# scwolof/gp_grief

Measured on AMD Instinct MI355X. Metric: CG iters/sec + Kron-matvec achieved HBM GB/s, 4D RBF grid 200^4, higher is better.
Workload: dtype f64

## Files before the change

### gp_grief_amd/csrc/gg_internal.h

```cpp
#pragma once

#include <hip/hip_runtime.h>

#include <algorithm>
#include <cstdint>
#include <cstdio>
#include <stdexcept>
#include <string>
#include <vector>

#include "../../include/gp_grief_amd.h"

namespace gg {

struct Error : std::runtime_error {
  int code;
  Error(int c, const std::string& m) : std::runtime_error(m), code(c) {}
};

void set_last_error(const std::string& msg);

#define GG_HIP(expr)                                                              \
  do {                                                                            \
    hipError_t e_ = (expr);                                                       \
    if (e_ != hipSuccess)                                                         \
      throw ::gg::Error(GG_ERR_RUNTIME, std::string("HIP error '") +              \
                                           hipGetErrorString(e_) + "' at " +     \
                                           __FILE__ + ":" + std::to_string(__LINE__) + \
                                           " in " #expr);                         \
  } while (0)

#define GG_REQUIRE(cond, code, msg)                 \
  do {                                              \
    if (!(cond)) throw ::gg::Error((code), (msg));  \
  } while (0)

template <class F>
int guard(F&& body) {
  try {
    body();
    return GG_OK;
  } catch (const Error& e) {
    set_last_error(e.what());
    return e.code;
  } catch (const std::bad_alloc&) {
    set_last_error("host allocation failed");
    return GG_ERR_RUNTIME;
  } catch (const std::exception& e) {
    set_last_error(e.what());
    return GG_ERR_RUNTIME;
  }
}

inline hipStream_t as_stream(gg_stream s) { return reinterpret_cast<hipStream_t>(s); }

#define GG_LAUNCH_CHECK() GG_HIP(hipGetLastError())

constexpr int kWave = 64;

inline int64_t ceil_div(int64_t a, int64_t b) { return (a + b - 1) / b; }

inline bool aligned16(const void* p) { return (reinterpret_cast<uintptr_t>(p) & 15) == 0; }

inline void check_status(int st) {
  if (st == GG_OK) return;
  char buf[512];
  gg_last_error(buf, sizeof buf);
  throw Error(st, buf);
}

constexpr int kXWinMax = 8;
constexpr int kXWinDefault = 8;
struct CgScalars {
  double rho;
  double rho_prev;
  double pq;
  double alpha;
  double beta;
  double tol;
  double bnorm;
  int iters;
  int done;
  int first;
  int pending;
  double rq, qq;
  int repair;
  int xpend;
  double xc[2];
  const double* xp[2];
  int xh;
  int xs;
  double xsc;
  const double* xsp;
  int cancels;
  double cancel_tol;
  int wk;
  int wn;
  int wnext;
  int warm;
  int wa[kXWinMax];
  double wc[kXWinMax + 1];
  const double* wp[kXWinMax + 1];
  int sreg, scnt;
  double scoef[kXWinMax];
  const double* sdir[kXWinMax];
  double beta_p;
  int rstored;
  const double* rp_cur;
  const double* rp_prev;
};

struct MpFuse {
  double* r = nullptr;
  const double* q_old = nullptr;
  double qshift = 0.0;
  double* p_out = nullptr;
  const CgScalars* sc = nullptr;
  double* rr_part = nullptr;
  int64_t rr_cap = 0;
  int64_t* pro_blocks = nullptr;
  int64_t pqo_stride = 0;
  double* sx = nullptr;
  const double* sp = nullptr;
  int64_t sn = 0, schunk = 0;
  int xdefer = 0;
  int xwin = 0;
  int64_t soff = 0;
  int64_t soff_h1 = 0, sn_h1 = 0;
  double* first_dst = nullptr;
  const double* er = nullptr;
  int64_t pstride = 0;
  double* ep_out = nullptr;
  double* ex = nullptr;
  const double* coef = nullptr;
  double* blk_q_out = nullptr;
  bool rderive = false;
  const double* pprev = nullptr;
};

struct OutMap {
  int identity;
  int64_t cg, gs, mi, cr, hs, as;
  int push = 0;
  int64_t self_off = 0;
  double* const* peers = nullptr;
  static OutMap ident() { return OutMap{1, 1, 0, 1, 1, 0, 0}; }
};

constexpr int kVecBlocks = 2048;
constexpr int kVecThreads = 256;

inline int vec_blocks(int64_t n) {
  const int64_t want = ceil_div(std::max<int64_t>(n / 2, 1), kVecThreads);
  return (int)std::min<int64_t>(kVecBlocks, std::max<int64_t>(want, 1));
}

struct KronDiag {
  int d;
  int64_t m[16];
  int64_t off[16];
};

inline KronDiag make_diag(int d, const int64_t* m, int64_t* n_out) {
  GG_REQUIRE(d >= 1 && d <= 16, GG_ERR_VALUE, "1 <= d <= 16 factors supported");
  GG_REQUIRE(m != nullptr, GG_ERR_VALUE, "NULL argument");
  KronDiag kd{};
  kd.d = d;
  int64_t n = 1, off = 0;
  for (int k = 0; k < d; ++k) {
    GG_REQUIRE(m[k] >= 1, GG_ERR_VALUE, "empty factor");
    kd.m[k] = m[k];
    kd.off[k] = off;
    off += m[k];
    n *= m[k];
  }
  *n_out = n;
  return kd;
}

// ... 125 lines not shown
```

### gp_grief_amd/csrc/gg_kronb.hip

```cpp
#include <algorithm>
#include <cmath>
#include <cstdlib>
#include <vector>

#include "gg_internal.h"

namespace gg {

typedef double bd4 __attribute__((ext_vector_type(4)));

constexpr int kBlkMaxD = 6;
constexpr int kBlkModeWaves = 12;
constexpr int kBlkPairWaves = 4;

struct BlockOp {
  int d = 0;
  int64_t m[kBlkMaxD] = {}, h[kBlkMaxD] = {};
  int64_t e[kBlkMaxD] = {};
  int64_t nb = 0, n = 0;
  double* frag[kBlkMaxD][2] = {};
  int KS[kBlkMaxD] = {}, JT[kBlkMaxD] = {};
  bool T4[kBlkMaxD] = {};
  int pTF = 0;
  int cus = 256;
// ... 682 lines not shown
#pragma unroll
        for (int r = 0; r < 4; ++r)
          stq(cvalid, a.Y, (cbase + (int64_t)(16 * t + 4 * r) * a.inner) * 8, o_e, acc[t][r]);
      stq(cvalid, a.Y, (cbase + (int64_t)16 * TF * a.inner) * 8, o_e, acc4);
      cur_next(cc);
    }
    sg0 = sg1;
  }
  if (KIND == 1 || KIND == 4) {
    __shared__ double red[2 * W];
#pragma unroll
    for (int off = 32; off > 0; off >>= 1) {
      rr_acc += __shfl_xor(rr_acc, off, 64);
      pqo_acc += __shfl_xor(pqo_acc, off, 64);
    }
    if (lane == 0) {
      red[wave] = rr_acc;
      red[W + wave] = pqo_acc;
    }
    __syncthreads();
    if (threadIdx.x == 0) {
      double s0 = 0.0, s1 = 0.0;
      for (int w = 0; w < W; ++w) {
        s0 += red[w];
        s1 += red[W + w];
      }
      if (a.rr_part != nullptr) {
        a.rr_part[blockIdx.x] = s0;
        if (a.pqo_stride > 0) a.rr_part[a.pqo_stride + blockIdx.x] = s1;
      }
    }
  }
}

struct PairArgs {
  const double* X;
  double* Y;
  const double* f3S;
  const double* f3T;
  const double* f2S;
  const double* f2T;
  int64_t nslab;
  int64_t spb;
  int64_t blk0;
  const double* P;
  double shift;
  double* partials;
  int64_t pstride;
  const int* skip;
  const CgScalars* sc;
  double* sx;
  int64_t soff, sn, soff_h1, sn_h1, sstep;
  int64_t sreg_len;
};

template <int R>
__device__ __forceinline__ double bcast_group(double v) {
  constexpr int pat = (R << 7) | 0x13;
  const int lo = __builtin_amdgcn_ds_swizzle(__double2loint(v), pat);
  const int hi = __builtin_amdgcn_ds_swizzle(__double2hiint(v), pat);
  return __hiloint2double(hi, lo);
}

template <int TF, int J0, int NJ, bool TJ, int EPI = -1, int PF = 4, bool NT = false>
__device__ __forceinline__ void pair_gemm2(const PairArgs& A, int64_t sbyte, const double* f2,
                                           const bd4 (&W)[TF][NJ > 0 ? NJ : 1],
                                           const double (&Wta)[NJ > 0 ? NJ : 1],
                                           const double (&Wj)[TF], const double Wc, double& pq,
                                           double& qq) {
  constexpr int H = 16 * TF + 4;
  constexpr int KS = 4 * TF + 1;
  constexpr int64_t FS = (int64_t)(TF + 1) * 64 * 8;
  const int lane = threadIdx.x & 63;
  const int n16 = lane & 15, kq = lane >> 4, l3 = lane & 3, b4 = (lane >> 2) & 3;
  uint32_t o_f = (uint32_t)(lane * 8);
  uint32_t o_z = (uint32_t)(((n16 >> 2) * 4 * H + 4 * kq + (n16 & 3)) * 8);
  uint32_t o_zt = (uint32_t)((16 * b4 + 4 * kq + l3) * 8);
  asm volatile("" : "+v"(o_f), "+v"(o_z), "+v"(o_zt));
  auto zb = [&](int i0, int a0) -> int64_t { return sbyte + ((int64_t)a0 * H + 4 * i0) * 8; };
  const bool epi = EPI < 0 ? A.P != nullptr : EPI != 0;
  const double sh = A.shift;
  auto bfull = [&](int s, int u) -> double {
    return s < 4 * TF ? W[s >> 2][u][s & 3] : Wta[u];
  };
  auto btail = [&](int s) -> double {
    if (s >= 4 * TF) return Wc;
    switch (s & 3) {
      case 0: return bcast_group<0>(Wj[s >> 2]);
      case 1: return bcast_group<1>(Wj[s >> 2]);
      case 2: return bcast_group<2>(Wj[s >> 2]);
      default: return bcast_group<3>(Wj[s >> 2]);
    }
  };
  auto put = [&](int64_t ub, uint32_t vo, double z, double p) {
    double q = z;
    if (epi) {
      q = fma(sh, p, q);
      pq = fma(p, q, pq);
      qq = fma(q, q, qq);
    }
    stuq<NT>(A.Y, ub, vo, q);
  };
#pragma unroll 1
  for (int ti = 0; ti < TF; ++ti) {
    bd4 Z[NJ > 0 ? NJ : 1];
    double Zt = 0.0;
#pragma unroll
// ... 319 lines not shown
  __shared__ __attribute__((aligned(16))) double ring[NS * R::STAGE];
  if (A.skip != nullptr && *A.skip) return;
  const int lane = threadIdx.x & 63;
  const int wave = __builtin_amdgcn_readfirstlane(threadIdx.x >> 6);
  const int sl = wave >> 1;
  const int64_t G = gridDim.x;
  const int64_t nunit = A.nslab / SPW;
  const int nmine = __builtin_amdgcn_readfirstlane(
      (int)((nunit - (int64_t)blockIdx.x + G - 1) / G));
  uint32_t dlane[R::DPW];
  uint32_t dlds[R::DPW];
#pragma unroll
  for (int j = 0; j < R::DPW; ++j) {
    const int i = wave * R::DPW + j;
    if (i < SPW * R::XI) {
      const int xs = i / R::XI, xi = i % R::XI;
      const int t = 2 * xi + (lane >> 5);
      const int row = min(16 * t + (lane & 15), H - 1);
      dlane[j] = (uint32_t)(xs * SB + (row * 4 + 2 * ((lane >> 4) & 1)) * 8);
      dlds[j] = (uint32_t)(xs * R::XD + xi * 128);
    } else {
      const int f = min(i - SPW * R::XI, R::FI - 1);
      dlane[j] = (uint32_t)((2 * f * 64 + 2 * lane) * 8);
      dlds[j] = (uint32_t)(R::FD + f * 128);
    }
  }
  auto src_at = [&](int it) {
    const int64_t slab = ((int64_t)blockIdx.x + (int64_t)it * G) * SPW;
    PairSlabSrc p;
    p.xoff = uni64(slab * SB);
    const int par = __builtin_amdgcn_readfirstlane((int)((slab / A.spb + A.blk0) & 1));
    p.f3 = par ? A.f3T : A.f3S;
    return p;
  };
  auto issue = [&](const PairSlabSrc& p, int st, int slot) {
    const char* xb = ubase(A.X, p.xoff + (int64_t)st * H * 32);
    const char* fbs = ubase(p.f3, (int64_t)st * FSK);
    double* dst = ring + slot * R::STAGE;
#pragma unroll
    for (int j = 0; j < R::DPW; ++j) {
      const int i = wave * R::DPW + j;
      const char* src = i < SPW * R::XI ? xb : fbs;
      __builtin_amdgcn_global_load_lds(
          reinterpret_cast<const __attribute__((address_space(1))) void*>(
              reinterpret_cast<uintptr_t>(src + dlane[j])),
          (__attribute__((address_space(3))) void*)(dst + dlds[j]), 16, 0, 0);
    }
  };
  double sc0 = 0.0, sc1 = 0.0;
  const double* sp0 = nullptr;
  const double* sp1 = nullptr;
  double* sxo = nullptr;
  int64_t slen = 0;
  double wcf[kXWinMax];
  const double* wdir[kXWinMax];
  int wcnt = 0;
  if (SIDE & 4) {
    if (A.sc->warm && !A.sc->done) {
      const int64_t off = (int64_t)A.sc->sreg * A.sreg_len;
      slen = max((int64_t)0, min(A.sn - off, A.sreg_len));
      wcnt = A.sc->scnt;
#pragma unroll
      for (int t = 0; t < kXWinMax; ++t) {
        wcf[t] = A.sc->scoef[t];
        wdir[t] = A.sc->sdir[t] + off;
      }
      sxo = A.sx + off;
    }
  } else if (SIDE & 1) {
    const int xh = A.sc->xh;
    if (xh < 2 && !A.sc->done) {
      const int64_t off = xh ? A.soff_h1 : A.soff;
      slen = xh ? A.sn_h1 : A.sn;
      sc0 = A.sc->xc[0];
      sc1 = A.sc->xc[1];
      sp0 = A.sc->xp[0] + off;
      sp1 = A.sc->xp[1] + off;
      sxo = A.sx + off;
    }
  }
  auto side_chunk = [&](int64_t slot) {
    const int64_t q0 = slot * A.sstep;
    const int64_t q1 = min(slen, q0 + A.sstep);
    constexpr int kSB = 16;
    for (int64_t e0 = q0 + 2 * lane; e0 < q1; e0 += kSB * 128) {
      double2 xv[kSB], a[kSB], b[kSB];
#pragma unroll
      for (int u = 0; u < kSB; ++u) {
        const int64_t e = e0 + (int64_t)u * 128;
        if (e + 1 < q1) {
          xv[u] = ld2g(sxo + e);
          a[u] = ld2g(sp0 + e);
          b[u] = ld2g(sp1 + e);
        }
      }
#pragma unroll
      for (int u = 0; u < kSB; ++u) {
        const int64_t e = e0 + (int64_t)u * 128;
        if (e + 1 < q1) {
          double2 o;
          o.x = xv[u].x + (sc0 * a[u].x + sc1 * b[u].x);
          o.y = xv[u].y + (sc0 * a[u].y + sc1 * b[u].y);
          st2g(sxo + e, o);
        }
      }
    }
  };
  auto side_chunk_win = [&](int64_t slot) {
    const int64_t q0 = slot * A.sstep;
    const int64_t q1 = min(slen, q0 + A.sstep);
    constexpr int kWB = 4;
    for (int64_t e0 = q0 + 2 * lane; e0 < q1; e0 += kWB * 128) {
      double2 xv[kWB], a[kXWinMax][kWB];
#pragma unroll
      for (int u = 0; u < kWB; ++u) {
        const int64_t e = e0 + (int64_t)u * 128;
        if (e + 1 < q1) xv[u] = ld2g(sxo + e);
      }
#pragma unroll
      for (int t = 0; t < kXWinMax; ++t)
        if (t < wcnt)
#pragma unroll
          for (int u = 0; u < kWB; ++u) {
            const int64_t e = e0 + (int64_t)u * 128;
            if (e + 1 < q1) a[t][u] = ld2g(wdir[t] + e);
          }
#pragma unroll
      for (int u = 0; u < kWB; ++u) {
        const int64_t e = e0 + (int64_t)u * 128;
        if (e + 1 < q1) {
          double2 s = {0.0, 0.0};
#pragma unroll
          for (int t = 0; t < kXWinMax; ++t)
            if (t < wcnt) {
              s.x += wcf[t] * a[t][u].x;
              s.y += wcf[t] * a[t][u].y;
            }
          double2 o;
          o.x = xv[u].x + s.x;
          o.y = xv[u].y + s.y;
          st2g(sxo + e, o);
        }
      }
    }
  };
  PairSlabSrc cur = src_at(0);
#pragma unroll
  for (int j = 0; j + 1 < NS; ++j) issue(cur, min(j, R::KS - 1), j);
  double pq = 0.0, qq = 0.0;
  int cslot = 0;
  for (int it = 0; it < nmine; ++it) {
    const int64_t slab = ((int64_t)blockIdx.x + (int64_t)it * G) * SPW + sl;
    const bool nv = it + 1 < nmine;
    const PairSlabSrc nxt = nv ? src_at(it + 1) : cur;
    const int role = (wave + it) & 1;
    if (role == 0)
      pair_slab_lds<TF, SPW, EPI, 0, JA, true, (SIDE & 2) != 0>(A, slab, sl, cslot, it == 0, cur, nxt, nv, ring,
                                               issue, pq, qq);
    else
      pair_slab_lds<TF, SPW, EPI, JA, TF - JA, false, (SIDE & 2) != 0>(A, slab, sl, cslot, it == 0, cur, nxt, nv,
                                                      ring, issue, pq, qq);
    if ((SIDE & 4) && slen > 0)
      side_chunk_win(((int64_t)blockIdx.x + (int64_t)it * G) * R::NW + wave);
    else if ((SIDE & 1) && slen > 0)
      side_chunk(((int64_t)blockIdx.x + (int64_t)it * G) * R::NW + wave);
    cslot = (cslot + R::KS) % NS;
    cur = nxt;
  }
  blk_wait_vm<0>();
  if (A.partials != nullptr) {
    __syncthreads();
    double* red = ring;
#pragma unroll
    for (int off = 32; off > 0; off >>= 1) {
      pq += __shfl_xor(pq, off, 64);
      qq += __shfl_xor(qq, off, 64);
    }
    if (lane == 0) {
      red[wave] = pq;
      red[R::NW + wave] = qq;
    }
    __syncthreads();
    if (threadIdx.x == 0) {
      double s0 = 0.0, s1 = 0.0;
      for (int w = 0; w < R::NW; ++w) {
        s0 += red[w];
        s1 += red[R::NW + w];
      }
      A.partials[blockIdx.x] = s0;
      A.partials[A.pstride + blockIdx.x] = 0.0;
      A.partials[2 * A.pstride + blockIdx.x] = s1;
    }
  }
}

typedef void (*blk_mode_fn)(ModeArgs);
typedef void (*blk_pair_fn)(PairArgs);



template <int KIND>
static blk_mode_fn mode_fn(int JT, bool T4) {
#define GG_BLK_MODE(jt)                                                    \
  case jt:                                                                 \
    return T4 ? blk_mode_kernel<jt, true, KIND> : blk_mode_kernel<jt, false, KIND>;
  switch (JT) {
    GG_BLK_MODE(1)
    GG_BLK_MODE(2)
    GG_BLK_MODE(3)
    GG_BLK_MODE(4)
    GG_BLK_MODE(5)
    GG_BLK_MODE(6)
    GG_BLK_MODE(7)
    default: return nullptr;
  }
#undef GG_BLK_MODE
}
// ... 378 lines not shown
      a.rr_part = cg->rr_part;
      GG_REQUIRE(grid <= cg->rr_cap, GG_ERR_VALUE, "prologue partial array too short");
      if (cg->pro_blocks != nullptr) *cg->pro_blocks = grid;
    } else if (kind == 2) {
      a.sc = cg->sc;
      a.sx = cg->sx;
      const int64_t sn = cg->sn;
      const int64_t H = block_side_half(sn);
      a.soff = 0;
      a.sn = std::min(H, sn);
      a.soff_h1 = a.sn;
      a.sn_h1 = sn - a.sn;
      const int64_t slots = a.ngroups * W;
      a.sstep = 2 * ceil_div(std::max<int64_t>(std::max(a.sn, a.sn_h1), 1), 2 * slots);
      GG_REQUIRE(a.sstep <= 128 * (int64_t)a.KS, GG_ERR_VALUE,
                 "block CG: x side job larger than its k-steps");
    }
    const blk_mode_fn fn = select_mode(kind, B->JT[k], B->T4[k], (int)B->h[k], B->fast);
    const size_t lds = (size_t)B->KS[k] * B->JT[k] * 64 * sizeof(double);
    hipLaunchKernelGGL(fn, dim3(grid), dim3(64 * W), lds, stream, a);
    GG_LAUNCH_CHECK();
    if (k == 0 && d == 3 && side && !pair_side)
      launch_x_half(cg->sx, cg->sn, block_side_half(cg->sn), cg->sc, stream);
    if (ev) GG_HIP(hipEventRecord(ev[++pos], stream));
    src = chain;
  }
  PairArgs p{};
  p.X = src;
  p.Y = cgp >= 2 ? cg->blk_q_out : y;
  const int k3 = d - 1, k2 = d - 2;
  p.f3S = B->frag[k3][0];
  p.f3T = B->frag[k3][1];
  p.f2S = B->frag[k2][0];
  p.f2T = B->frag[k2][1];
  p.spb = B->nb / (B->e[k3] * B->e[k2]);
  p.nslab = p.spb * nblk;
  p.blk0 = blk0;
  p.skip = skip;
  const int grid = pair_grid(B, nblk);
  if (cgp >= 2) {
    p.P = cg->p_out;
    p.shift = shift;
    p.partials = dot_partials;
    p.pstride = cg->pstride;
  } else if (shift != 0.0) {
    p.P = x;
    p.shift = shift;
  }
  if (pair_side && win) {
    p.sc = cg->sc;
    p.sx = cg->sx;
    p.sn = cg->sn;
    p.sreg_len = xwin_region(cg->sn, cg->xwin);
    const int64_t slots = p.nslab / B->pair_spw * 2 * B->pair_spw;
    p.sstep = 2 * ceil_div(std::max<int64_t>(p.sreg_len, 1), 2 * slots);
  } else if (pair_side) {
    p.sc = cg->sc;
    p.sx = cg->sx;
    const int64_t sn = cg->sn;
    const int64_t H = block_side_half(sn);
    p.soff = 0;
    p.sn = std::min(H, sn);
    p.soff_h1 = p.sn;
    p.sn_h1 = sn - p.sn;
    const int64_t slots = p.nslab / B->pair_spw * 2 * B->pair_spw;
    p.sstep = 2 * ceil_div(std::max<int64_t>(std::max(p.sn, p.sn_h1), 1), 2 * slots);
  }
  hipLaunchKernelGGL(select_pair(B->pTF, B->pair_lds, B->pair_spw, p.P != nullptr, pair_side,
                                 B->epi_nt && (pair_side || cgp == 3), win),
                     dim3(grid), dim3(B->pair_lds ? 128 * B->pair_spw : 64 * kBlkPairWaves), 0,
                     stream, p);
  GG_LAUNCH_CHECK();
  if (ev) GG_HIP(hipEventRecord(ev[++pos], stream));
  if (n_partials) *n_partials = (cgp >= 2) ? grid : 0;
}

int64_t block_side_half(int64_t n) { return 2 * ceil_div(n, (int64_t)4); }

bool block_pair_side(const BlockOp* B) { return B != nullptr && B->pair_lds; }

bool block_rderive_ok(const BlockOp* B) {
  if (B == nullptr || B->d < 3 || !B->pro_nt) return false;
  const int JT = B->JT[0];
  return B->T4[0] && B->h[0] == 16 * (JT - 1) + 4 && B->fast && mode_fast_fn<5>(JT) != nullptr;
}

bool block_efficient(const BlockOp* B) {
  if (B == nullptr) return false;
  const int d = B->d;
  return B->e[d - 1] == B->h[d - 1] && B->e[d - 2] == B->h[d - 2];
}

}
```

### gp_grief_amd/csrc/gg_vec.hip

```cpp
#include <cmath>
#include <map>
#include <vector>

#include "gg_internal.h"

namespace gg {

__global__ __launch_bounds__(kVecThreads) void dot_partials_kernel(const double* __restrict__ x,
                                                                   const double* __restrict__ y,
                                                                   int64_t n,
                                                                   double* __restrict__ partials) {
  double acc = 0.0;
  const int64_t stride = (int64_t)gridDim.x * blockDim.x;
  const int64_t n2 = n / 2;
  const double2* x2 = reinterpret_cast<const double2*>(x);
  const double2* y2 = reinterpret_cast<const double2*>(y);
  for (int64_t i = (int64_t)blockIdx.x * blockDim.x + threadIdx.x; i < n2; i += stride) {
    const double2 a = x2[i], b = y2[i];
    acc = fma(a.x, b.x, acc);
    acc = fma(a.y, b.y, acc);
  }
  if (blockIdx.x == 0 && threadIdx.x == 0 && (n & 1)) acc = fma(x[n - 1], y[n - 1], acc);
  const double s = block_sum(acc);
  if (threadIdx.x == 0) partials[blockIdx.x] = s;
// ... 454 lines not shown
    sc->wnext = 0;
    sc->warm = 0;
    for (int r = 0; r < kXWinMax; ++r) sc->wa[r] = 0;
    sc->beta_p = 0.0;
    sc->rstored = 1;
    sc->rp_cur = sc->rp_prev = nullptr;
    sc->done = (s == 0.0 || !(sqrt(s) >= sc->tol)) ? 1 : 0;
  }
}

void scalars_clear(CgScalars* sc) {
  GG_HIP(hipMemset(sc, 0, sizeof(CgScalars)));
  const char* e = knob("GG_CG_CANCEL_TOL");
  if (e) {
    const double t = atof(e);
    GG_HIP(hipMemcpy(&sc->cancel_tol, &t, sizeof(double), hipMemcpyHostToDevice));
  }
}
}

struct gg_cg {
  const gg_kron* K = nullptr;
  double shift = 0.0;
  int64_t n = 0;
  double *r = nullptr, *p = nullptr, *q = nullptr, *mv_work = nullptr;
  double* p2 = nullptr;
  double* p3 = nullptr;
  double* p4 = nullptr;
  double* first_dst = nullptr;
  bool fused = true;
  int fusion = 0;
  int xdefer = 2;
  double* partials = nullptr;
  double* rr_part = nullptr;
  int64_t rr_count = 0;
  int rq = 1;
  gg::CgScalars* sc = nullptr;
  gg::CgScalars* sc_host = nullptr;
  const double* b = nullptr;
  double* x = nullptr;
  int64_t mv_partials = 0;
  bool await_finish = false;
  bool profiling = false;
  std::vector<hipEvent_t> events;
  size_t events_used = 0;
  const gg::BlockOp* blk = nullptr;
  int basis = 1;
  bool block = false;
  double* xb = nullptr;
  double* q2 = nullptr;
  int64_t rblk0 = 0, rnblk = -1;
  bool restart = false;
  int xwin = 0;
  int xmode = 0;
  double* ring[gg::kXWinMax + 1] = {};
  int pcur = 0;
  double *q_c = nullptr, *q2_c = nullptr;
  bool rder_ok = true;
  bool rder = false;
  double* pprev_buf() const {
    const int ns = nring();
    return ring[(pcur + ns - 1) % ns];
  }
  int launches() const { return block ? gg::block_launches(blk) : gg::kron_d(K); }
  int nring() const { return xmode == 3 ? xwin + 1 : 4; }
  int64_t nvec() const { return (block && rnblk < 0) ? gg::block_n(blk) : n; }
  void reset_buffers() {
    p = ring[0];
    p2 = ring[1];
    p3 = ring[2];
    p4 = ring[3];
    q = q_c;
    q2 = q2_c;
    pcur = 0;
  }
  void rotate_dirs() {
    if (xmode == 3) {
      const int ns = nring();
      pcur = (pcur + 1) % ns;
      p = ring[pcur];
      p2 = ring[(pcur + 1) % ns];
    } else if (xmode == 2) {
      double* cur = p;
      double* o2 = p3;
      p = p2;
      p2 = p4;
      p3 = cur;
      p4 = o2;
    } else if (xmode == 1) {
      double* old_ = p3;
      p3 = p;
      p = p2;
      p2 = old_;
    } else {
      std::swap(p, p2);
    }
  }
};

namespace gg {
static int cg_xwin_knob() {
  const char* e = knob("GG_CG_XWIN");
  const int k = e ? atoi(e) : kXWinDefault;
  return k < 2 ? 0 : std::min(k, kXWinMax);
}
static int64_t cg_extra_dirs(int K) { return K >= 2 ? std::max(0, K + 1 - 4) : 0; }
int64_t xwin_region(int64_t n, int K) { return 2 * ceil_div(n, 2 * (int64_t)K); }
}

extern "C" {

int gg_dot(const double* x_dev, const double* y_dev, int64_t n, double* out_host,
           gg_stream stream) {
  return gg::guard([&] {
    GG_REQUIRE(x_dev && y_dev && out_host && n >= 0, GG_ERR_VALUE, "bad argument");
    hipStream_t s = gg::as_stream(stream);
    double* buf = nullptr;
    GG_HIP(hipMallocAsync(&buf, (gg::kVecBlocks + 1) * sizeof(double), s));
    const int nb = gg::vec_blocks(n);
    if (gg::aligned16(x_dev) && gg::aligned16(y_dev)) {
      gg::launch_dot_partials(x_dev, y_dev, n, buf, nb, s);
    } else {
      hipLaunchKernelGGL(gg::dot_partials_unaligned_kernel, dim3(nb), dim3(gg::kVecThreads), 0,
                         s, x_dev, y_dev, n, buf);
      GG_LAUNCH_CHECK();
    }
    gg::launch_reduce_to(buf, nb, buf + gg::kVecBlocks, s);
    GG_HIP(hipMemcpyAsync(out_host, buf + gg::kVecBlocks, sizeof(double),
                          hipMemcpyDeviceToHost, s));
    GG_HIP(hipFreeAsync(buf, s));
    GG_HIP(hipStreamSynchronize(s));
  });
}

int gg_axpby(double a, const double* x_dev, double b, double* y_dev, int64_t n,
             gg_stream stream) {
  return gg::guard([&] {
    GG_REQUIRE(x_dev && y_dev && n >= 0, GG_ERR_VALUE, "bad argument");
    if (n == 0) return;
    hipLaunchKernelGGL(gg::axpby_kernel, dim3(gg::vec_blocks(2 * n)), dim3(gg::kVecThreads),
                       0, gg::as_stream(stream), a, x_dev, b, y_dev, n);
    GG_LAUNCH_CHECK();
  });
}

static int64_t cg_vec_pad() {
  const char* e = gg::knob("GG_CG_VEC_PAD");
  const int64_t v = e ? atoll(e) : 0;
  return v > 0 ? 2 * (v / 2) : 0;
}
static int64_t cg_vec_stride(int64_t n) { return (n + 31) / 32 * 32 + cg_vec_pad(); }
constexpr int64_t kCgAlignSlack = 32;

static int64_t cg_layout_elems(const gg_kron* K, int64_t n, int64_t* extra_off = nullptr,
                               int* xwin = nullptr, int64_t* vstride = nullptr) {
  const gg::BlockOp* B = gg::kron_block(K);
  const int64_t vs = cg_vec_stride(B ? std::max(n, gg::block_n(B)) : n);
// ... 9 lines not shown
static thread_local std::map<const gg_kron*, int64_t> t_cg_sized;

int gg_cg_work_elems(const gg_kron* K, int64_t* elems) {
  return gg::guard([&] {
    GG_REQUIRE(K && elems, GG_ERR_VALUE, "NULL argument");
    gg::knobs_reload();
    const int64_t n = gg::kron_n(K);
    *elems = cg_layout_elems(K, n);
    t_cg_sized[K] = *elems;
  });
}

int gg_cg_work_elems_blocks(const gg_kron* K, int64_t nblk, int64_t* elems) {
  return gg::guard([&] {
    GG_REQUIRE(K && elems, GG_ERR_VALUE, "NULL argument");
    const gg::BlockOp* B = gg::kron_block(K);
    GG_REQUIRE(B != nullptr, GG_ERR_VALUE, "the operator has no parity-block basis");
    GG_REQUIRE(nblk >= 1 && nblk <= ((int64_t)1 << gg::block_d(B)), GG_ERR_VALUE,
               "block count outside 1..2^d");
    gg::knobs_reload();
    const int w = gg::block_pair_side(B) ? gg::cg_xwin_knob() : 0;
    *elems = kCgAlignSlack + (7 + gg::cg_extra_dirs(w)) * cg_vec_stride(nblk * gg::block_nb(B));
  });
}

int gg_cg_create_blocks(const gg_kron* K, int64_t blk0, int64_t nblk, double shift,
                        double* work_dev, gg_cg** out) {
  return gg::guard([&] {
    GG_REQUIRE(K && work_dev && out, GG_ERR_VALUE, "NULL argument");
    const gg::BlockOp* B = gg::kron_block(K);
    GG_REQUIRE(B != nullptr, GG_ERR_VALUE, "the operator has no parity-block basis");
    GG_REQUIRE(gg::block_d(B) >= 3, GG_ERR_VALUE, "the block-sharded CG needs d >= 3");
    GG_REQUIRE(blk0 >= 0 && nblk >= 1 && blk0 + nblk <= ((int64_t)1 << gg::block_d(B)),
               GG_ERR_VALUE, "block range outside the 2^d blocks");
    GG_REQUIRE((reinterpret_cast<uintptr_t>(work_dev) & 15) == 0, GG_ERR_VALUE,
               "the CG workspace must be 16-byte aligned");
    const int64_t n = nblk * gg::block_nb(B);
    gg_cg* cg = new gg_cg();
    try {
      cg->K = K;
      cg->shift = shift;
      cg->n = n;
      const int64_t vs = cg_vec_stride(n);
      work_dev = reinterpret_cast<double*>((reinterpret_cast<uintptr_t>(work_dev) + 255) &
                                           ~static_cast<uintptr_t>(255));
      cg->r = work_dev;
      cg->p = work_dev + vs;
      cg->q = work_dev + 2 * vs;
      cg->p2 = work_dev + 3 * vs;
      cg->p3 = work_dev + 4 * vs;
      cg->p4 = work_dev + 5 * vs;
      cg->q2 = work_dev + 6 * vs;
      cg->xwin = gg::block_pair_side(B) ? gg::cg_xwin_knob() : 0;
      cg->ring[0] = cg->p;
      cg->ring[1] = cg->p2;
      cg->ring[2] = cg->p3;
      cg->ring[3] = cg->p4;
      for (int i = 0; i < gg::cg_extra_dirs(cg->xwin); ++i) cg->ring[4 + i] = work_dev + (7 + i) * vs;
      cg->q_c = cg->q;
      cg->q2_c = cg->q2;
      cg->blk = B;
      cg->basis = 1;
      cg->rblk0 = blk0;
      cg->rnblk = nblk;
      cg->fused = true;
      const char* rde = gg::knob("GG_CG_RDERIVE");
      cg->rder_ok = !(rde && atoi(rde) == 0);
      cg->mv_partials = gg::block_partials_needed(B);
      GG_HIP(hipMalloc(&cg->partials,
                       std::max<int64_t>(gg::kVecBlocks, 3 * cg->mv_partials) * sizeof(double)));
      cg->rr_count = gg::block_prologue_blocks(B);
      GG_HIP(hipMalloc(&cg->rr_part, 2 * cg->rr_count * sizeof(double)));
      GG_HIP(hipMemset(cg->rr_part, 0, 2 * cg->rr_count * sizeof(double)));
      GG_HIP(hipMalloc(&cg->sc, sizeof(gg::CgScalars)));
      GG_HIP(hipHostMalloc(&cg->sc_host, sizeof(gg::CgScalars), hipHostMallocDefault));
      gg::scalars_clear(cg->sc);
    } catch (...) {
      gg_cg_destroy(cg);
      throw;
    }
    *out = cg;
  });
}

int gg_cg_create(const gg_kron* K, double shift, double* work_dev, gg_cg** out) {
  return gg::guard([&] {
    GG_REQUIRE(K && work_dev && out, GG_ERR_VALUE, "NULL argument");
    int64_t nr = 0, nc = 0, we = 0;
    gg_kron_shape(K, 0, &nr, &nc, &we);
    GG_REQUIRE(nr == nc, GG_ERR_VALUE, "CG needs a square operator");
    gg_cg* cg = new gg_cg();
    try {
      cg->K = K;
      cg->shift = shift;
      cg->n = nr;
      int64_t vs = 0;
      const int64_t need = cg_layout_elems(K, nr, nullptr, nullptr, &vs);
      const auto sized = t_cg_sized.find(K);
      GG_REQUIRE(sized == t_cg_sized.end() || need <= sized->second, GG_ERR_VALUE,
                 "the CG workspace was sized (gg_cg_work_elems) under another GG_* snapshot: "
                 "call gg_cg_work_elems again before gg_cg_create");
      if (sized != t_cg_sized.end()) t_cg_sized.erase(sized);
      GG_REQUIRE((reinterpret_cast<uintptr_t>(work_dev) & 7) == 0, GG_ERR_VALUE,
                 "the CG workspace must hold doubles (8-byte aligned)");
      const bool base16 = (reinterpret_cast<uintptr_t>(work_dev) & 15) == 0;
      work_dev = reinterpret_cast<double*>((reinterpret_cast<uintptr_t>(work_dev) + 255) &
                                           ~static_cast<uintptr_t>(255));
      cg->r = work_dev;
      cg->p = work_dev + vs;
      cg->q = work_dev + 2 * vs;
      cg->p2 = work_dev + 3 * vs;
      cg->p3 = work_dev + 4 * vs;
      cg->p4 = work_dev + 5 * vs;
      cg->mv_work = work_dev + 6 * vs;
      if (gg::kron_d(K) % 2 == 1) cg->first_dst = cg->mv_work + gg::kron_work_elems(K, false);
      cg->blk = gg::kron_block(K);
      int64_t extra_off = 0;
      int xwin = 0;
      cg_layout_elems(K, nr, &extra_off, &xwin);
      cg->ring[0] = cg->p;
      cg->ring[1] = cg->p2;
      cg->ring[2] = cg->p3;
      cg->ring[3] = cg->p4;
      cg->q_c = cg->q;
      if (cg->blk != nullptr) {
        cg->xb = work_dev + 6 * vs;
        cg->q2 = work_dev + 7 * vs;
        cg->q2_c = cg->q2;
        const char* be = gg::knob("GG_CG_BASIS");
        cg->basis = be ? (atoi(be) != 0 ? 1 : 0) : (gg::block_efficient(cg->blk) ? 1 : 0);
        cg->xwin = gg::block_pair_side(cg->blk) ? xwin : 0;
        for (int i = 0; i < gg::cg_extra_dirs(xwin); ++i)
          cg->ring[4 + i] = work_dev + extra_off + i * vs;
      } else {
        cg->basis = 0;
      }
      const char* xd = gg::knob("GG_CG_XDEFER");
      if (xd) cg->xdefer = std::min(2, std::max(0, atoi(xd)));
      const char* rqe = gg::knob("GG_CG_RQ");
      if (rqe) cg->rq = std::min(2, std::max(0, atoi(rqe)));
      const char* rse = gg::knob("GG_CG_RESTART");
      cg->restart = rse && atoi(rse) == 1;
      const char* rde = gg::knob("GG_CG_RDERIVE");
      cg->rder_ok = !(rde && atoi(rde) == 0);
      cg->mv_partials = gg::kron_partials_needed(K, false);
      if (cg->blk) cg->mv_partials = std::max(cg->mv_partials, gg::block_partials_needed(cg->blk));
      const int64_t np = std::max<int64_t>(gg::kVecBlocks, 3 * cg->mv_partials);
      GG_HIP(hipMalloc(&cg->partials, np * sizeof(double)));
      cg->fused = gg::kron_d(K) >= 2 && (nr % 2) == 0 && base16;
      if (cg->fused) {
        cg->rr_count = gg::kron_prologue_blocks(K);
        if (cg->blk) cg->rr_count = std::max(cg->rr_count, gg::block_prologue_blocks(cg->blk));
        GG_HIP(hipMalloc(&cg->rr_part, 2 * cg->rr_count * sizeof(double)));
        GG_HIP(hipMemset(cg->rr_part, 0, 2 * cg->rr_count * sizeof(double)));
      }
      GG_HIP(hipMalloc(&cg->sc, sizeof(gg::CgScalars)));
      GG_HIP(hipHostMalloc(&cg->sc_host, sizeof(gg::CgScalars), hipHostMallocDefault));
      gg::scalars_clear(cg->sc);
    } catch (...) {
      gg_cg_destroy(cg);
      throw;
    }
    *out = cg;
  });
}

int gg_cg_destroy(gg_cg* cg) {
  return gg::guard([&] {
    if (!cg) return;
    if (cg->partials) (void)hipFree(cg->partials);
    if (cg->rr_part) (void)hipFree(cg->rr_part);
    if (cg->sc) (void)hipFree(cg->sc);
    if (cg->sc_host) (void)hipHostFree(cg->sc_host);
    for (hipEvent_t e : cg->events) (void)hipEventDestroy(e);
    delete cg;
  });
}

int gg_cg_profile(gg_cg* cg, int enable) {
  return gg::guard([&] {
    GG_REQUIRE(cg, GG_ERR_VALUE, "NULL handle");
    cg->profiling = enable != 0;
    cg->events_used = 0;
  });
// ... 239 lines not shown
  return gg::guard([&] {
    GG_REQUIRE(cg && cg->x, GG_ERR_VALUE, "CG not started");
    GG_REQUIRE(cg->rnblk < 0, GG_ERR_VALUE,
               "a block-range handle (gg_cg_create_blocks) runs through gg_cg_iterate_partial");
    hipStream_t s = gg::as_stream(stream);
    const int64_t n = cg->nvec();
    const int nb = gg::vec_blocks(n);
    if (check_every <= 0) check_every = max_iters;
    for (int it = 0; it < max_iters; ++it) {
      int64_t nparts = 0;
      hipEvent_t* ev = nullptr;
      if (cg->profiling) {
        const size_t need = cg->events_used + (size_t)cg->launches() + 1;
        while (cg->events.size() < need) {
          hipEvent_t e;
          GG_HIP(hipEventCreate(&e));
          cg->events.push_back(e);
        }
        ev = cg->events.data() + cg->events_used;
        cg->events_used = need;
      }
      const int xmode = cg->xmode;
      const bool xdefer = xmode != 0;
      if (cg->fused) {
        if (!cg->restart) {
          if (cg->rder)
            hipLaunchKernelGGL(gg::cg_r_materialize_kernel, dim3(nb), dim3(gg::kVecThreads), 0,
                               s, cg->r, cg->q, n, cg->sc, cg->partials, 2);
          else
            hipLaunchKernelGGL(gg::cg_xr_update_kernel, dim3(nb), dim3(gg::kVecThreads), 0, s,
                               xdefer ? nullptr : cg->x, cg->r, cg->p, cg->q, n, cg->sc,
                               cg->partials, 2);
          GG_LAUNCH_CHECK();
          hipLaunchKernelGGL(gg::cg_rho_kernel, dim3(1), dim3(1024), 0, s, cg->partials,
                             (int64_t)nb, cg->sc, 2);
          GG_LAUNCH_CHECK();
        }
        gg::MpFuse fz;
        fz.r = cg->r;
        fz.q_old = cg->q;
        fz.p_out = cg->fusion == 0 ? cg->p2 : nullptr;
        fz.ep_out = cg->fusion == 0 ? nullptr : cg->p2;
        fz.ex = cg->fusion == 2 ? cg->x : nullptr;
        fz.sc = cg->sc;
        fz.rr_part = cg->rr_part;
        fz.rr_cap = cg->rr_count;
        int64_t pro_blocks = 0;
        fz.pro_blocks = &pro_blocks;
        fz.sx = cg->fusion == 2 ? nullptr : cg->x;
        fz.sp = cg->p;
        fz.sn = n;
        fz.xdefer = xmode;
        fz.xwin = cg->xwin;
        fz.rderive = cg->rder;
        fz.pprev = cg->rder ? cg->pprev_buf() : nullptr;
        fz.first_dst = cg->first_dst;
        const bool rq_ident = cg->rq != 0 && cg->fusion == 0;
        fz.er = (rq_ident && cg->rq != 2) ? nullptr : cg->r;
        fz.pqo_stride = rq_ident ? cg->rr_count : 0;
        fz.pstride = cg->mv_partials;
        if (cg->block) {
          fz.sx = cg->xb;
          fz.blk_q_out = cg->q2;
          gg::block_apply(cg->blk, cg->p, cg->q, cg->shift, nullptr, cg->partials,
                          &cg->sc->done, s, &nparts, &fz, 2, ev);
        } else {
          gg::kron_apply(cg->K, false, cg->p, cg->q, cg->shift, cg->mv_work, cg->partials,
                         &cg->sc->done, s, &nparts, &fz, 2, ev);
        }
        GG_REQUIRE(pro_blocks > 0 && pro_blocks <= cg->rr_count, GG_ERR_RUNTIME,
                   "fused CG: no prologue launch recorded");
        hipLaunchKernelGGL(gg::cg_fused_scalars_kernel, dim3(1), dim3(1024), 0, s, cg->rr_part,
                           pro_blocks, cg->rr_count, cg->partials, nparts, cg->mv_partials,
                           cg->sc,
                           xdefer ? (const double*)cg->p2 : nullptr, xmode, rq_ident ? 1 : 0,
                           cg->rder ? 1 : 0);
        GG_LAUNCH_CHECK();
        if (cg->block) std::swap(cg->q, cg->q2);
        cg->rotate_dirs();
      } else {
        gg::MpFuse fz;
        fz.r = cg->r;
        fz.sc = cg->sc;
        gg::kron_apply(cg->K, false, cg->p, cg->q, cg->shift, cg->mv_work, cg->partials,
                       &cg->sc->done, s, &nparts, &fz, 1, ev);
        hipLaunchKernelGGL(gg::cg_alpha_kernel, dim3(1), dim3(1024), 0, s, cg->partials, nparts,
                           cg->sc);
        GG_LAUNCH_CHECK();
        hipLaunchKernelGGL(gg::cg_xr_update_kernel, dim3(nb), dim3(gg::kVecThreads), 0, s,
                           cg->x, cg->r, cg->p, cg->q, n, cg->sc, cg->partials, 0);
        GG_LAUNCH_CHECK();
        hipLaunchKernelGGL(gg::cg_rho_kernel, dim3(1), dim3(1024), 0, s, cg->partials,
                           (int64_t)nb, cg->sc, 0);
        GG_LAUNCH_CHECK();
      }
      if ((it + 1) % check_every == 0 && it + 1 < max_iters) {
        GG_HIP(hipMemcpyAsync(cg->sc_host, cg->sc, sizeof(gg::CgScalars),
                              hipMemcpyDeviceToHost, s));
        GG_HIP(hipStreamSynchronize(s));
        if (cg->sc_host->done) break;
      }
    }
  });
}

int gg_cg_close(gg_cg* cg, gg_stream stream) {
// ... 71 lines not shown
    const int nb = gg::vec_blocks(n);
    gg::launch_dot_partials(cg->r, cg->r, n, cg->partials, nb, s);
    gg::launch_reduce_to(cg->partials, nb, rr_dev, s);
  });
}

int gg_cg_start_finish(gg_cg* cg, const double* rr_dev, double rtol, double atol,
                       gg_stream stream) {
  return gg::guard([&] {
    GG_REQUIRE(cg && cg->x && rr_dev, GG_ERR_VALUE, "CG not started (gg_cg_start_partial)");
    GG_REQUIRE(rtol >= 0 && atol >= 0, GG_ERR_VALUE,
               "tolerances must be real, non-negative numbers");
    hipLaunchKernelGGL(gg::cg_init_kernel, dim3(1), dim3(1024), 0, gg::as_stream(stream), rr_dev,
                       (int64_t)1, cg->sc, rtol, atol);
    GG_LAUNCH_CHECK();
  });
}

int gg_cg_iterate_partial(gg_cg* cg, double* red_dev, gg_stream stream) {
  return gg::guard([&] {
    GG_REQUIRE(cg && cg->x && red_dev, GG_ERR_VALUE, "CG not started");
    GG_REQUIRE(cg->fused && cg->fusion == 0, GG_ERR_VALUE,
               "the sharded rank runs the fused recurrence, layout 0");
    GG_REQUIRE(!cg->await_finish, GG_ERR_VALUE, "gg_cg_iterate_finish first");
    hipStream_t s = gg::as_stream(stream);
    const int64_t n = cg->n;
    int64_t nparts = 0;
    hipEvent_t* ev = nullptr;
    if (cg->profiling) {
      const size_t need = cg->events_used + (size_t)cg->launches() + 1;
      while (cg->events.size() < need) {
        hipEvent_t e;
        GG_HIP(hipEventCreate(&e));
        cg->events.push_back(e);
      }
      ev = cg->events.data() + cg->events_used;
      cg->events_used = need;
    }
    const int xmode = cg->xmode;
    gg::MpFuse fz;
    fz.r = cg->r;
    fz.q_old = cg->q;
    fz.p_out = cg->p2;
    fz.sc = cg->sc;
    fz.rr_part = cg->rr_part;
    fz.rr_cap = cg->rr_count;
    int64_t pro_blocks = 0;
    fz.pro_blocks = &pro_blocks;
    fz.sx = cg->x;
    fz.sp = cg->p;
    fz.sn = n;
    fz.xdefer = xmode;
    fz.xwin = cg->xwin;
    fz.rderive = cg->rder;
    fz.pprev = cg->rder ? cg->pprev_buf() : nullptr;
    fz.first_dst = cg->first_dst;
    const bool rq_ident = cg->rq != 0;
    fz.er = rq_ident ? nullptr : cg->r;
    fz.pqo_stride = rq_ident ? cg->rr_count : 0;
    fz.pstride = cg->mv_partials;
    if (cg->block) {
      fz.blk_q_out = cg->q2;
      gg::block_apply(cg->blk, cg->p, cg->q, cg->shift, nullptr, cg->partials, &cg->sc->done, s,
                      &nparts, &fz, 2, ev, cg->rblk0, cg->rnblk);
    } else {
      gg::kron_apply(cg->K, false, cg->p, cg->q, cg->shift, cg->mv_work, cg->partials,
                     &cg->sc->done, s, &nparts, &fz, 2, ev);
    }
    GG_REQUIRE(pro_blocks > 0 && pro_blocks <= cg->rr_count, GG_ERR_RUNTIME,
               "fused CG: no prologue launch recorded");
    if (cg->block) std::swap(cg->q, cg->q2);
    hipLaunchKernelGGL(gg::cg_local_red_kernel, dim3(1), dim3(1024), 0, s, cg->rr_part,
                       pro_blocks, cg->rr_count, cg->partials, nparts, cg->mv_partials,
                       rq_ident ? 1 : 0, red_dev);
    GG_LAUNCH_CHECK();
    cg->await_finish = true;
  });
}

int gg_cg_iterate_finish(gg_cg* cg, const double* red_dev, gg_stream stream) {
  return gg::guard([&] {
    GG_REQUIRE(cg && red_dev, GG_ERR_VALUE, "NULL argument");
    GG_REQUIRE(cg->await_finish, GG_ERR_VALUE, "gg_cg_iterate_partial first");
    hipStream_t s = gg::as_stream(stream);
    const int xmode = cg->xmode;
    const bool rq_ident = cg->rq != 0;
    hipLaunchKernelGGL(gg::cg_fused_scalars_kernel, dim3(1), dim3(1024), 0, s, red_dev,
                       (int64_t)1, (int64_t)1, red_dev + 2, (int64_t)1, (int64_t)1, cg->sc,
                       xmode ? (const double*)cg->p2 : nullptr, xmode, rq_ident ? 1 : 0,
                       cg->rder ? 1 : 0);
    GG_LAUNCH_CHECK();
    cg->rotate_dirs();
    cg->await_finish = false;
  });
}

int gg_cg_close_partial(gg_cg* cg, double* rr_dev, gg_stream stream) {
  return gg::guard([&] {
    GG_REQUIRE(cg && cg->x && rr_dev, GG_ERR_VALUE, "CG not started");
    GG_REQUIRE(!cg->await_finish, GG_ERR_VALUE, "gg_cg_iterate_finish first");
    hipStream_t s = gg::as_stream(stream);
    const int64_t n = cg->n;
    const int nb = gg::vec_blocks(n);
    if (cg->xmode == 3) {
      hipLaunchKernelGGL(gg::cg_x_flush3_kernel, dim3(nb), dim3(gg::kVecThreads), 0, s, cg->x, n,
                         gg::xwin_region(n, cg->xwin), cg->sc);
// ... 71 lines not shown
```

Measured before the change: 31.53.

## Batch windowed x-update side work into periodic software-pipelined phases

Instead of interleaving a small x-window update chunk after every pair slab, each block now accumulates its share and runs a larger phase every few slabs (default 8), staggered across blocks by CU. The phase is specialized at compile time on the window count, issues deep software-pipelined loads with clamped addresses, and writes out-of-range lanes to a trash buffer. Coefficients and direction pointers are fetched with scalar loads inside the phase rather than kept in registers across the main loop. This aims to cut register pressure and improve memory-level parallelism of the side stream, at the cost of burstier HBM traffic and a new requirement that n be even.

```diff
diff --git a/gp_grief_amd/csrc/gg_internal.h b/gp_grief_amd/csrc/gg_internal.h
--- a/gp_grief_amd/csrc/gg_internal.h
+++ b/gp_grief_amd/csrc/gg_internal.h
@@ -71,6 +71,8 @@
 
 constexpr int kXWinMax = 8;
 constexpr int kXWinDefault = 8;
+constexpr int kXWinPhaseMax = 8;
+constexpr int kXWinPhaseDefault = 8;
 struct CgScalars {
   double rho;
   double rho_prev;
@@ -125,6 +127,7 @@
   int64_t sn = 0, schunk = 0;
   int xdefer = 0;
   int xwin = 0;
+  int xphase = 0;
   int64_t soff = 0;
   int64_t soff_h1 = 0, sn_h1 = 0;
   double* first_dst = nullptr;
diff --git a/gp_grief_amd/csrc/gg_kronb.hip b/gp_grief_amd/csrc/gg_kronb.hip
--- a/gp_grief_amd/csrc/gg_kronb.hip
+++ b/gp_grief_amd/csrc/gg_kronb.hip
@@ -758,7 +758,26 @@
   double* sx;
   int64_t soff, sn, soff_h1, sn_h1, sstep;
   int64_t sreg_len;
+  int sphase;
+  int scus;
 };
+
+__device__ __forceinline__ void sld8(const void* p, uint64_t (&v)[8]) {
+  asm volatile(
+      "s_load_dwordx2 %0, %8, 0x0\n\t"
+      "s_load_dwordx2 %1, %8, 0x8\n\t"
+      "s_load_dwordx2 %2, %8, 0x10\n\t"
+      "s_load_dwordx2 %3, %8, 0x18\n\t"
+      "s_load_dwordx2 %4, %8, 0x20\n\t"
+      "s_load_dwordx2 %5, %8, 0x28\n\t"
+      "s_load_dwordx2 %6, %8, 0x30\n\t"
+      "s_load_dwordx2 %7, %8, 0x38\n\t"
+      "s_waitcnt lgkmcnt(0)"
+      : "=&s"(v[0]), "=&s"(v[1]), "=&s"(v[2]), "=&s"(v[3]), "=&s"(v[4]), "=&s"(v[5]),
+        "=&s"(v[6]), "=&s"(v[7])
+      : "s"(p)
+      : "memory");
+}
 
 template <int R>
 __device__ __forceinline__ double bcast_group(double v) {
@@ -1184,20 +1203,14 @@
   const double* sp1 = nullptr;
   double* sxo = nullptr;
   int64_t slen = 0;
-  double wcf[kXWinMax];
-  const double* wdir[kXWinMax];
+  int64_t woff = 0;
   int wcnt = 0;
   if (SIDE & 4) {
     if (A.sc->warm && !A.sc->done) {
-      const int64_t off = (int64_t)A.sc->sreg * A.sreg_len;
-      slen = max((int64_t)0, min(A.sn - off, A.sreg_len));
+      woff = (int64_t)A.sc->sreg * A.sreg_len;
+      slen = max((int64_t)0, min(A.sn - woff, A.sreg_len));
       wcnt = A.sc->scnt;
-#pragma unroll
-      for (int t = 0; t < kXWinMax; ++t) {
-        wcf[t] = A.sc->scoef[t];
-        wdir[t] = A.sc->sdir[t] + off;
-      }
-      sxo = A.sx + off;
+      sxo = A.sx + woff;
     }
   } else if (SIDE & 1) {
     const int xh = A.sc->xh;
@@ -1242,6 +1255,16 @@
     const int64_t q0 = slot * A.sstep;
     const int64_t q1 = min(slen, q0 + A.sstep);
     constexpr int kWB = 4;
+    uint64_t dc[8], dd[8];
+    sld8(A.sc->scoef, dc);
+    sld8(A.sc->sdir, dd);
+    double wcf[kXWinMax];
+    const double* wdir[kXWinMax];
+#pragma unroll
+    for (int t = 0; t < kXWinMax; ++t) {
+      wcf[t] = __longlong_as_double((long long)dc[t]);
+      wdir[t] = reinterpret_cast<const double*>(dd[t]) + woff;
+    }
     for (int64_t e0 = q0 + 2 * lane; e0 < q1; e0 += kWB * 128) {
       double2 xv[kWB], a[kXWinMax][kWB];
 #pragma unroll
@@ -1276,6 +1299,91 @@
       }
     }
   };
+  auto win_phase = [&](auto wc_tag, int64_t p0, int64_t p1) {
+    constexpr int WC = decltype(wc_tag)::value;
+    constexpr int D = WC >= 6 ? 4 : WC >= 4 ? 6 : 8;
+    constexpr int64_t kStride = (int64_t)R::NW * 128;
+    uint64_t dc[8], dd[8];
+    sld8(A.sc->scoef, dc);
+    sld8(A.sc->sdir, dd);
+    double cf[WC];
+    const double* dir[WC];
+#pragma unroll
+    for (int t = 0; t < WC; ++t) {
+      cf[t] = __longlong_as_double((long long)dc[t]);
+      dir[t] = reinterpret_cast<const double*>(dd[t]) + woff;
+    }
+    const int64_t last = p1 - 2;
+    int ln = lane;
+    asm volatile("" : "+v"(ln));
+    double* const trash = g_blk_trash + 2 * ln;
+    double2 xv[D], a[D][WC];
+    auto load = [&](int j, int64_t eb) {
+      const int64_t ebc = min(eb, last);
+      const uint32_t vo = (uint32_t)min((int64_t)(2 * ln), last - ebc) * 8u;
+      {
+        const gchar* b = reinterpret_cast<const gchar*>(
+            reinterpret_cast<uintptr_t>(ubase(sxo, ebc * 8)));
+        const gd2v v = *reinterpret_cast<const gd2*>(b + vo);
+        xv[j] = double2{v.x, v.y};
+      }
+#pragma unroll
+      for (int t = 0; t < WC; ++t) {
+        const gchar* b = reinterpret_cast<const gchar*>(
+            reinterpret_cast<uintptr_t>(ubase(dir[t], ebc * 8)));
+        const gd2v v = *reinterpret_cast<const gd2*>(b + vo);
+        a[j][t] = double2{v.x, v.y};
+      }
+      __builtin_amdgcn_sched_barrier(0);
+    };
+    auto finish = [&](int j, int64_t eb) {
+      double2 s = {0.0, 0.0};
+#pragma unroll
+      for (int t = 0; t < WC; ++t) {
+        s.x += cf[t] * a[j][t].x;
+        s.y += cf[t] * a[j][t].y;
+      }
+      double2 o;
+      o.x = xv[j].x + s.x;
+      o.y = xv[j].y + s.y;
+      const int64_t e = eb + 2 * ln;
+      st2g(e + 1 < p1 ? sxo + e : trash, o);
+      __builtin_amdgcn_sched_barrier(0);
+    };
+    const int64_t e0 = p0 + (int64_t)wave * 128;
+#pragma unroll
+    for (int j = 0; j < D; ++j) load(j, e0 + j * kStride);
+#pragma unroll 1
+    for (int64_t eb = e0; eb < p1; eb += D * kStride) {
+#pragma unroll
+      for (int j = 0; j < D; ++j) {
+        finish(j, eb + j * kStride);
+        load(j, eb + (j + D) * kStride);
+      }
+    }
+  };
+  auto win_phase_n = [&](int64_t p0, int64_t p1) {
+    if (p0 >= p1) return;
+    switch (wcnt) {
+      case 1: win_phase(std::integral_constant<int, 1>(), p0, p1); break;
+      case 2: win_phase(std::integral_constant<int, 2>(), p0, p1); break;
+      case 3: win_phase(std::integral_constant<int, 3>(), p0, p1); break;
+      case 4: win_phase(std::integral_constant<int, 4>(), p0, p1); break;
+      case 5: win_phase(std::integral_constant<int, 5>(), p0, p1); break;
+      case 6: win_phase(std::integral_constant<int, 6>(), p0, p1); break;
+      case 7: win_phase(std::integral_constant<int, 7>(), p0, p1); break;
+      case 8: win_phase(std::integral_constant<int, 8>(), p0, p1); break;
+      default: break;
+    }
+  };
+  const int wR = (SIDE & 4) ? A.sphase : 1;
+  int64_t ufirst = 0;
+  int pdone = 0, pctr = 0;
+  if ((SIDE & 4) && wR >= 2) {
+    const int64_t ub = nunit / G, ur = nunit % G;
+    ufirst = (int64_t)blockIdx.x * ub + min((int64_t)blockIdx.x, ur);
+    pctr = (int)((blockIdx.x / 8 + blockIdx.x / (unsigned)max(A.scus, 1)) % (unsigned)wR);
+  }
   PairSlabSrc cur = src_at(0);
 #pragma unroll
   for (int j = 0; j + 1 < NS; ++j) issue(cur, min(j, R::KS - 1), j);
@@ -1292,9 +1400,18 @@
     else
       pair_slab_lds<TF, SPW, EPI, JA, TF - JA, false, (SIDE & 2) != 0>(A, slab, sl, cslot, it == 0, cur, nxt, nv,
                                                       ring, issue, pq, qq);
-    if ((SIDE & 4) && slen > 0)
-      side_chunk_win(((int64_t)blockIdx.x + (int64_t)it * G) * R::NW + wave);
-    else if ((SIDE & 1) && slen > 0)
+    if ((SIDE & 4) && slen > 0) {
+      if (wR < 2) {
+        side_chunk_win(((int64_t)blockIdx.x + (int64_t)it * G) * R::NW + wave);
+      } else {
+        pctr = pctr + 1 == wR ? 0 : pctr + 1;
+        if (pctr == 0 || !nv) {
+          win_phase_n(min(slen, (ufirst + pdone) * A.sstep),
+                      min(slen, (ufirst + it + 1) * A.sstep));
+          pdone = it + 1;
+        }
+      }
+    } else if ((SIDE & 1) && slen > 0)
       side_chunk(((int64_t)blockIdx.x + (int64_t)it * G) * R::NW + wave);
     cslot = (cslot + R::KS) % NS;
     cur = nxt;
@@ -1779,8 +1896,16 @@
     p.sx = cg->sx;
     p.sn = cg->sn;
     p.sreg_len = xwin_region(cg->sn, cg->xwin);
-    const int64_t slots = p.nslab / B->pair_spw * 2 * B->pair_spw;
-    p.sstep = 2 * ceil_div(std::max<int64_t>(p.sreg_len, 1), 2 * slots);
+    GG_REQUIRE(cg->sn % 2 == 0, GG_ERR_VALUE, "block CG: the x window takes x in pairs");
+    p.sphase = cg->xphase >= 1 && cg->xphase <= kXWinPhaseMax ? cg->xphase : kXWinPhaseDefault;
+    p.scus = B->cus;
+    const int64_t units = p.nslab / B->pair_spw;
+    if (p.sphase >= 2) {
+      p.sstep = 16 * ceil_div(std::max<int64_t>(p.sreg_len, 1), 16 * units);
+    } else {
+      const int64_t slots = units * 2 * B->pair_spw;
+      p.sstep = 2 * ceil_div(std::max<int64_t>(p.sreg_len, 1), 2 * slots);
+    }
   } else if (pair_side) {
     p.sc = cg->sc;
     p.sx = cg->sx;
diff --git a/gp_grief_amd/csrc/gg_vec.hip b/gp_grief_amd/csrc/gg_vec.hip
--- a/gp_grief_amd/csrc/gg_vec.hip
+++ b/gp_grief_amd/csrc/gg_vec.hip
@@ -530,6 +530,7 @@
   int64_t rblk0 = 0, rnblk = -1;
   bool restart = false;
   int xwin = 0;
+  int xphase = 0;
   int xmode = 0;
   double* ring[gg::kXWinMax + 1] = {};
   int pcur = 0;
@@ -581,6 +582,11 @@
   const char* e = knob("GG_CG_XWIN");
   const int k = e ? atoi(e) : kXWinDefault;
   return k < 2 ? 0 : std::min(k, kXWinMax);
+}
+static int cg_xphase_knob() {
+  const char* e = knob("GG_CG_XWIN_PHASE");
+  const int r = e ? atoi(e) : kXWinPhaseDefault;
+  return std::min(std::max(r, 1), kXWinPhaseMax);
 }
 static int64_t cg_extra_dirs(int K) { return K >= 2 ? std::max(0, K + 1 - 4) : 0; }
 int64_t xwin_region(int64_t n, int K) { return 2 * ceil_div(n, 2 * (int64_t)K); }
@@ -696,6 +702,7 @@
       cg->p4 = work_dev + 5 * vs;
       cg->q2 = work_dev + 6 * vs;
       cg->xwin = gg::block_pair_side(B) ? gg::cg_xwin_knob() : 0;
+      cg->xphase = gg::cg_xphase_knob();
       cg->ring[0] = cg->p;
       cg->ring[1] = cg->p2;
       cg->ring[2] = cg->p3;
@@ -774,6 +781,7 @@
         const char* be = gg::knob("GG_CG_BASIS");
         cg->basis = be ? (atoi(be) != 0 ? 1 : 0) : (gg::block_efficient(cg->blk) ? 1 : 0);
         cg->xwin = gg::block_pair_side(cg->blk) ? xwin : 0;
+        cg->xphase = gg::cg_xphase_knob();
         for (int i = 0; i < gg::cg_extra_dirs(xwin); ++i)
           cg->ring[4 + i] = work_dev + extra_off + i * vs;
       } else {
@@ -1119,6 +1127,7 @@
         fz.sn = n;
         fz.xdefer = xmode;
         fz.xwin = cg->xwin;
+    fz.xphase = cg->xphase;
         fz.rderive = cg->rder;
         fz.pprev = cg->rder ? cg->pprev_buf() : nullptr;
         fz.first_dst = cg->first_dst;
@@ -1296,6 +1305,7 @@
     fz.sn = n;
     fz.xdefer = xmode;
     fz.xwin = cg->xwin;
+    fz.xphase = cg->xphase;
     fz.rderive = cg->rder;
     fz.pprev = cg->rder ? cg->pprev_buf() : nullptr;
     fz.first_dst = cg->first_dst;
```

Result: faster. 31.85 (median of 6 runs) (+1.0%).
